# cambridge-mlg/RECOMBINER

Measured on AMD Instinct MI355X. Metric: INRs trained/sec (whole node) + PSNR@bpp vs reference, CIFAR-10, higher is better.
Workload: dtype bf16; 1 GPU; CIFAR-10 32x32, 4096 INRs/GPU, 3x32 SIREN (in 32 = 16 Fourier + 16 upsampled pe), S=1, training_mappings=True, Adam lr 2e-4; inrs_per_gpu=4096, parallelism=datapoint-sharded x1, tuned_library_gemms=True

## Files before the change

include/rcb.h:

```cpp
#ifndef RCB_H_
#define RCB_H_

#include <stdint.h>

#ifdef __cplusplus
extern "C" {
#endif

#define RCB_VERSION 407
#define RCB_OK 0
#define RCB_ERR_ARG (-1)
#define RCB_ERR_SHAPE (-2)
#define RCB_ERR_UNSUPPORTED (-3)
#define RCB_KL_SLOTS 1024
#define RCB_KL_FX_SCALE 16777216.0

typedef void* rcb_stream_t;

int rcb_version(void);
const char* rcb_last_error_string(void);
#define RCB_STRUCT_SIREN_DESC 0
#define RCB_STRUCT_LEVEL 1
#define RCB_STRUCT_LEVEL_BWD 2
#define RCB_STRUCT_ADAM_CFG 3
#define RCB_STRUCT_ADAM_TENSOR 4
#define RCB_STRUCT_REC_DESC 5
int64_t rcb_struct_bytes(int32_t which);

typedef struct {
  int32_t n_rows;
  int32_t samples;
  int32_t n_pix;
// ... 193 lines not shown
} rcb_rec_desc;

int64_t rcb_rec_workspace_bytes(int32_t n_jobs, int32_t max_glen, int32_t n_candidates);
int rcb_rec_score_argmax(const rcb_rec_desc* desc, int32_t mode, void* workspace, int64_t workspace_bytes, int32_t* idx,
                         double* best, uint8_t* uncertified, double* logw_job0, rcb_stream_t stream);
int rcb_rec_commit(const rcb_rec_desc* desc, const int32_t* idx, const int32_t* job_group, int32_t n_groups,
                   double* z_out, float* enc_sample, float* enc_mask, uint8_t* done, float* beta,
                   int32_t* idx_groupwise, rcb_stream_t stream);

int rcb_upconv_fwd(const void* x, int32_t x_is_f32_preact, const float* weff, const float* bias, void* y,
                   int32_t y_is_f32_linear, int32_t batch, int32_t grid, int32_t cout, const void* frag_pack,
                   rcb_stream_t stream);
int32_t rcb_upconv_dgrad_partial_rows(int32_t batch);
int rcb_upconv_dgrad(const void* dy, int32_t dy_is_f32, const float* weff, const void* x, int32_t x_is_f32_preact,
                     void* dx, float* dbias_partial, int32_t batch, int32_t grid, int32_t cout, const void* frag_pack,
                     rcb_stream_t stream);
int64_t rcb_upconv_wgrad_workspace(int32_t batch, int32_t cout);
int rcb_upconv_wgrad(const void* x, int32_t x_is_f32_preact, const void* dy, int32_t dy_is_f32, float* dweff,
                     float* dbias, int32_t batch, int32_t grid, int32_t cout, float* workspace,
                     int64_t workspace_floats, rcb_stream_t stream);
int rcb_upconv_bwd_fused(const void* dy, const float* weff, const void* x, void* dx, float* dweff, float* dbias,
                         int32_t batch, int32_t grid, int32_t cout, float* workspace, int64_t workspace_floats,
                         const void* frag_pack, rcb_stream_t stream);

#define RCB_UPCONV_PACK_UINT4 22528
int rcb_upconv_weff_build(const float* W1, const float* b1, const float* W2, const float* W3, void* weff1, void* b1rep,
                          int32_t bf16_out, float* weff2, float* weff3, void* frag_pack, rcb_stream_t stream);
int rcb_upconv_weff_grad(const void* dweff1, int32_t bf16_in, const float* dweff2, const float* dweff3, float* dW1,
                         float* dW2, float* dW3, const float* db1_partial ,
                         int32_t n_partial, float* db1 ,
                         rcb_stream_t stream);

int rcb_tile_gather(const void* img, void* tiles, int32_t n, int32_t H, int32_t W, int32_t C, int32_t Ty, int32_t Tx,
                    int32_t T, int32_t step, int32_t off, int32_t ring, rcb_stream_t stream);
int rcb_tile_crop(const void* tiles, void* img, int32_t n, int32_t H, int32_t W, int32_t C, int32_t Ty, int32_t Tx,
                  int32_t T, int32_t off, rcb_stream_t stream);
int rcb_tile_fold(const void* tiles, void* img, int32_t n, int32_t H, int32_t W, int32_t C, int32_t Ty, int32_t Tx,
                  int32_t T, int32_t off, rcb_stream_t stream);

int64_t rcb_phaseconv_pack_uint4(int32_t nd, int32_t cout, int32_t which);
int rcb_phaseconv_pack(const float* conv_weight, int32_t nd, int32_t cout, void* fwd_frags, void* dgrad_frags,
                       rcb_stream_t stream);
int rcb_phaseconv_fwd(const void* x, const void* fwd_frags, const float* bias, void* y, int32_t B, int32_t g0, int32_t g1,
                      int32_t g2, int32_t nd, int32_t cout, int32_t leaky_out, rcb_stream_t stream);
int rcb_phaseconv_dgrad(const void* dy, const void* dgrad_frags, const void* x_act, void* dx, int32_t B, int32_t g0,
                        int32_t g1, int32_t g2, int32_t nd, int32_t cout, rcb_stream_t stream);
// ... 27 lines not shown
```

recombiner_amd/_lib.py:

```python
import ctypes as C
import os

import torch

_HERE = os.path.dirname(os.path.abspath(__file__))
LIB_PATH = os.environ.get("RCB_LIB") or os.path.join(_HERE, "lib", "librcb_hip.so")

class RcbError(RuntimeError):
    pass


class SirenDesc(C.Structure):
    _fields_ = [("n_rows", C.c_int32), ("samples", C.c_int32), ("n_pix", C.c_int32), ("fourier_dim", C.c_int32),
                ("pe_dim", C.c_int32), ("n_hidden", C.c_int32), ("hidden", C.c_int32), ("out_dim", C.c_int32),
                ("xf_inr_stride", C.c_int64), ("w_row_stride", C.c_int64), ("w0", C.c_float),
                ("precision", C.c_int32), ("pe_bf16", C.c_int32), ("dw_bf16", C.c_void_p), ("pixel_chunks", C.c_int32),
                ("xf_bf16", C.c_void_p), ("pe_grid_dims", C.c_int32), ("pe_patch_nums", C.c_int32 * 3),
                ("pe_patch_size", C.c_int32 * 3), ("dw_bf16_stride", C.c_int64), ("hidden_dims", C.c_int32 * 4),
                ("dw_lo", C.c_void_p), ("clock_probe", C.c_void_p)]


class Level(C.Structure):
    _fields_ = [("loc", C.c_void_p), ("log_scale", C.c_void_p), ("enc_sample", C.c_void_p),
                ("enc_mask", C.c_void_p), ("row_map", C.c_void_p), ("row_perm", C.c_void_p),
# ... 14 lines not shown


class AdamCfg(C.Structure):
    _fields_ = [("lr", C.c_float), ("beta1", C.c_float), ("beta2", C.c_float), ("eps", C.c_float),
                ("step", C.c_int32), ("dyn_scalars", C.c_void_p)]


class LevelBwd(C.Structure):
    _fields_ = [("loc", C.c_void_p), ("log_scale", C.c_void_p), ("enc_mask", C.c_void_p), ("p_loc", C.c_void_p),
                ("p_scale", C.c_void_p), ("p_scale_is_log", C.c_int32), ("beta", C.c_void_p),
                ("group_idx", C.c_void_p), ("n_groups", C.c_int32), ("kl_scalar", C.c_float),
                ("d_out", C.c_void_p), ("eps", C.c_void_p), ("member_ptr", C.c_void_p),
                ("member_idx", C.c_void_p), ("row_perm_inv", C.c_void_p), ("col_inv", C.c_void_p),
                ("rows", C.c_int32), ("cols", C.c_int32), ("cols_out", C.c_int32), ("samples", C.c_int32),
                ("g_loc", C.c_void_p), ("g_log_scale", C.c_void_p), ("m_loc", C.c_void_p), ("v_loc", C.c_void_p),
                ("m_ls", C.c_void_p), ("v_ls", C.c_void_p), ("kl_accum", C.c_void_p), ("kl_scalar_dev", C.c_void_p),
                ("next_out", C.c_void_p), ("next_eps", C.c_void_p), ("next_out_bf16", C.c_void_p),
                ("next_ld_bf16", C.c_int64), ("rng_seed", C.c_uint64), ("rng_step_dev", C.c_void_p),
                ("rng_step_add", C.c_int64), ("rng_stream", C.c_uint32), ("eps_from_rng", C.c_uint32),
                ("rng_group_offset", C.c_uint64), ("next_out_lo", C.c_void_p), ("sample_sum_ws", C.c_void_p), ("col_map", C.c_void_p)]


_lib = None
ABI_VERSION = 407
_MIRRORS = {0: SirenDesc, 1: Level, 2: LevelBwd, 3: AdamCfg, 4: AdamTensor, 5: RecDesc}

_int, _i32, _i64, _u32, _u64, _f32, _f64, _p = C.c_int, C.c_int32, C.c_int64, C.c_uint32, C.c_uint64, C.c_float, C.c_double, C.c_void_p
_siren, _level, _level_bwd = C.POINTER(SirenDesc), C.POINTER(Level), C.POINTER(LevelBwd)
_adam_cfg, _adam_tensor, _rec = C.POINTER(AdamCfg), C.POINTER(AdamTensor), C.POINTER(RecDesc)
PROTOTYPES = {
    "rcb_version": (_int, []),
    "rcb_last_error_string": (C.c_char_p, []),
    "rcb_struct_bytes": (_i64, [_i32]),
    "rcb_debug_siren_wave_tiles": (_int, [_i32]),
    "rcb_siren_fwd": (_int, [_siren] + [_p] * 5),
    "rcb_siren_bwd": (_int, [_siren] + [_p] * 7),
    "rcb_siren_reduce_chunks": (_int, [_siren] + [_p] * 5),
    "rcb_siren_loss_bwd": (_int, [_siren, _p, _p, _p, _p, _f32, _p, _p, _p, _p]),
    "rcb_reparam_fwd": (_int, [_level, _i32, _i32, _i32, _i32, _p, _p]),
    "rcb_reparam_hier_rng_fwd": (_int, [_level, _i32, _i32, _i32, _p, _p, _u64, _p, _p, _u64, _p]),
    "rcb_philox_normal": (_int, [_p, _i64, _u64, _u32, _p, _i64, _u64, _p]),
    "rcb_reparam_rng_fwd": (_int, [_p, _p, _i64, _u64, _u32, _p, _p, _p, _p, _p, _i32, _i64, _u64, _p]),
    "rcb_gauss_kl": (_int, [_p, _p, _p, _p, _i32, _i32, _i32, _p, _p, _i32, _p, _p, _p, _p, _p]),
    "rcb_gauss_kl_colsum": (_int, [_p, _p, _i32, _p, _p, _i32, _i32, _p, _p]),
    "rcb_beta_update": (_int, [_p, _p, _p, _i32, _i32, _f64, _f64, _f64, _f64, _p]),
    "rcb_posterior_bwd": (_int, [_level_bwd, _adam_cfg, _p]),
    "rcb_adam_flat": (_int, [_p, _p, _p, _p, _i64, _adam_cfg, _p]),
# ... 1 lines not shown
    "rcb_debug_generic_kernels_only": (_int, [_i32]),
    "rcb_atrans_pack_elems": (_i64, [_i32, _p]),
    "rcb_atrans_pack": (_int, [_p, _i32, _p, _p, _i32, _p]),
    "rcb_atrans_plan": (_int, [_i64, _i32, _p, _i32, _p, _i32]),
    "rcb_atrans_apply": (_int, [_p, _i64, _p, _p, _i64, _p, _i64, _i64, _i32, _p, _p, _i32, _i32, _p, _p, _p, _p]),
    "rcb_atrans_workspace_floats": (_i64, [_i64, _i32, _p, _p]),
    "rcb_atrans_wgrad_narrow_workspace": (_i64, [_i32, _i32]),
    "rcb_atrans_wgrad_narrow": (_int, [_p, _p, _p, _i64, _p, _p, _p, _i64, _i64, _i32, _p, _p, _i32, _p]),
    "rcb_step_begin": (_int, [_p, _i64, _p, _p, _p, _p]),
    "rcb_step_end": (_int, [_p, _i32, _f64, _p, _p, _p, _i64, _p, _p, _p]),
    "rcb_step_prepare": (_int, [_p, _i64, _p, _p, _p, _p, _i32, _p, _p, _i32] + [_p] * 6 + [_i32, _p, _p, _p, _p]),
    "rcb_step_tail_eligible": (_int, [_level_bwd]),
    "rcb_step_tail": (_int, [_level_bwd, _adam_cfg, _adam_tensor, _i32, _p, _i32, _f64, _p, _p, _i64, _p, _p, _p, _p]),
    "rcb_col_moments": (_int, [_p, _p, _i32, _i32, _p, _p]),
    "rcb_rec_workspace_bytes": (_i64, [_i32, _i32, _i32]),
    "rcb_rec_score_argmax": (_int, [_rec, _i32, _p, _i64, _p, _p, _p, _p, _p]),
    "rcb_rec_commit": (_int, [_rec, _p, _p, _i32] + [_p] * 7),
    "rcb_upconv_fwd": (_int, [_p, _i32, _p, _p, _p, _i32, _i32, _i32, _i32, _p, _p]),
    "rcb_upconv_dgrad_partial_rows": (_i32, [_i32]),
    "rcb_upconv_dgrad": (_int, [_p, _i32, _p, _p, _i32, _p, _p, _i32, _i32, _i32, _p, _p]),
    "rcb_upconv_wgrad_workspace": (_i64, [_i32, _i32]),
    "rcb_upconv_wgrad": (_int, [_p, _i32, _p, _i32, _p, _p, _i32, _i32, _i32, _p, _i64, _p]),
    "rcb_upconv_bwd_fused": (_int, [_p] * 6 + [_i32, _i32, _i32, _p, _i64, _p, _p]),
    "rcb_upconv_weff_build": (_int, [_p] * 6 + [_i32, _p, _p, _p, _p]),
    "rcb_upconv_weff_grad": (_int, [_p, _i32, _p, _p, _p, _p, _p, _p, _i32, _p, _p]),
    "rcb_tile_gather": (_int, [_p, _p] + [_i32] * 10 + [_p]),
    "rcb_tile_crop": (_int, [_p, _p] + [_i32] * 8 + [_p]),
    "rcb_tile_fold": (_int, [_p, _p] + [_i32] * 8 + [_p]),
    "rcb_phaseconv_pack_uint4": (_i64, [_i32, _i32, _i32]),
    "rcb_phaseconv_pack": (_int, [_p, _i32, _i32, _p, _p, _p]),
    "rcb_phaseconv_fwd": (_int, [_p] * 4 + [_i32] * 7 + [_p]),
    "rcb_phaseconv_dgrad": (_int, [_p] * 4 + [_i32] * 6 + [_p]),
    "rcb_phaseconv_wgrad_workspace": (_i64, [_i32, _i32]),
    "rcb_phaseconv_wgrad": (_int, [_p] * 5 + [_i64] + [_i32] * 6 + [_p]),
    "rcb_stage1_1d_fwd": (_int, [_p, _p, _p, _p, _i32, _i32, _p]),
    "rcb_stage1_1d_dgrad": (_int, [_p, _p, _p, _i32, _i32, _p]),
    "rcb_stage1_1d_wgrad_workspace": (_i64, []),
    "rcb_stage1_1d_wgrad": (_int, [_p] * 5 + [_i64, _i32, _i32, _p]),
    "rcb_window_gather": (_int, [_p, _p] + [_i32] * 6 + [_p]),
    "rcb_window_fold": (_int, [_p, _p] + [_i32] * 6 + [_p]),
    "rcb_phase_bigweight": (_int, [_p, _p, _i32, _i32, _p, _i32, _i32, _i32, _i32, _p]),
    "rcb_phase_bigweight_grad": (_int, [_p, _i32, _p, _i32, _p, _i32, _i32, _i32, _i32, _p]),
    "rcb_softplus_scale": (_int, [_p, _p, _i64, _p]),
}
EXPORTS = list(PROTOTYPES)

# ... 52 lines not shown
```

recombiner_amd/csrc/upconv.hip:

```cpp
#include "rcb_common.h"

using namespace rcb;

typedef float f32x16 __attribute__((ext_vector_type(16)));
typedef __bf16 bf16x8 __attribute__((ext_vector_type(8)));
typedef __bf16 bf16x4 __attribute__((ext_vector_type(4)));
typedef short s16x4 __attribute__((ext_vector_type(4)));

namespace {

constexpr int CIN = 64;
#ifndef RCB_UP_HOT
#define RCB_UP_HOT 0
#endif
#ifndef RCB_UP_NOSTORE
#define RCB_UP_NOSTORE 0
#endif
#ifndef RCB_B3_PF
#define RCB_B3_PF 2
#endif
#ifndef RCB_UP_PF
#define RCB_UP_PF 3
#endif
constexpr int XRS = 72;
// ... 489 lines not shown
#pragma unroll
          for (int k = 0; k < 4; ++k) {
            o0.v[k] = (__bf16)xa[k];     o0.v[4 + k] = (__bf16)ya[k];
            o1.v[k] = (__bf16)xa[4 + k]; o1.v[4 + k] = (__bf16)ya[4 + k];
          }
          uint4* dst = reinterpret_cast<uint4*>(reinterpret_cast<__bf16*>(a.y) + opix * COUT + 32 * mt + 16 * h);
          if (RCB_UP_NOSTORE != 1 || a.batch < 0) {
            dst[0] = o0.u;
            dst[1] = o1.u;
          }
        }
        __builtin_amdgcn_sched_barrier(0);
        F2_T(4);
      }
    }
  }
#if RCB_F2_STAMPS
  ph_[6] = __builtin_amdgcn_s_memrealtime();
  ph_[7] = t_entry_;
  if (blockIdx.x == 0 && lane == 0)
    for (int k = 0; k < 8; ++k) g_f2_stamps[wave * 8 + k] = ph_[k];
#endif
#undef RCB_FETCH2
}

#ifndef RCB_D2_STAMPS
#define RCB_D2_STAMPS 0
#endif
#if RCB_D2_STAMPS
__device__ unsigned long long g_d2_stamps[8 * 8];
#define D2_T(k)                                                     \
  do {                                                              \
    const unsigned long long now_ = __builtin_amdgcn_s_memtime();   \
    ph_[k] += now_ - last_;                                         \
    last_ = now_;                                                   \
  } while (0)
#else
#define D2_T(k) do { } while (0)
#endif
template <int X_F32>
__global__ void __launch_bounds__(512) upconv_dgrad2_reg_kernel(DgradArgs a, float* __restrict__ dbias_partial) {
  constexpr int G = 8, OG = 16, HO = 18, RS = 64, ROWS = HO * RS + 32, COUT = 64, IMG = HO * ROWS;
#if RCB_D2_STAMPS
  const unsigned long long t_entry_ = __builtin_amdgcn_s_memrealtime();
#endif
  extern __shared__ __attribute__((aligned(16))) unsigned char smem_raw[];
// ... 816 lines not shown
}

extern "C" int rcb_upconv_bwd_fused(const void* dy, const float* weff, const void* x, void* dx, float* dweff, float* dbias,
                                    int32_t batch, int32_t grid, int32_t cout, float* workspace, int64_t workspace_floats,
                                    const void* frag_pack, rcb_stream_t stream) {
  RCB_REQUIRE(dy && weff && x && dx && dweff && workspace, RCB_ERR_ARG, "upconv_bwd_fused: null pointer");
  RCB_REQUIRE(batch > 0, RCB_ERR_SHAPE, "upconv_bwd_fused: empty batch");
  RCB_REQUIRE(grid == 16 && cout == 16, RCB_ERR_UNSUPPORTED, "upconv_bwd_fused: grid=%d cout=%d not instantiated", grid, cout);
  RCB_REQUIRE(workspace_floats >= rcb_upconv_wgrad_workspace(batch, cout), RCB_ERR_SHAPE,
              "upconv_bwd_fused: workspace of %lld floats, %lld needed", (long long)workspace_floats,
              (long long)rcb_upconv_wgrad_workspace(batch, cout));
  RCB_REQUIRE((reinterpret_cast<uintptr_t>(frag_pack) & 15) == 0, RCB_ERR_ARG, "upconv_bwd_fused: frag_pack must be 16-byte aligned");
  Bwd3Args a{dy, weff, x, dx, workspace, batch, reinterpret_cast<const uint4*>(frag_pack)};
  hipStream_t st = (hipStream_t)stream;
  const int g = wgrad_blocks(batch);
  static bool done = false;
  int rc = launch(upconv_bwd3_fused_kernel, a, g, 32 * 1024 + (34 * 34 * 24 + 18 * 18 * (RCB_B3_WG16 ? 64 : XRS)) * 2 + 8 * 32 * 40 * 2, st, done);
  if (rc) return rc;
  const int row = 1024 * cout + cout;
  upconv_wgrad_reduce_kernel<<<(row + 63) / 64, 256, 0, st>>>(workspace, g, row, 1024 * cout, dweff, dbias);
  RCB_LAUNCH_CHECK();
  return RCB_OK;
}
```

recombiner_amd/ops.py:

```python
import collections
import ctypes as C
import os as _os
from dataclasses import dataclass
from typing import List, Optional, Sequence

import numpy as np
import torch

from . import _lib
from ._lib import AdamCfg, AdamTensor, Level, LevelBwd, RcbError, SirenDesc, addr, check, ptr, stream_ptr

f32 = torch.float32
f64 = torch.float64
i32 = torch.int32
bf16 = torch.bfloat16


@dataclass(frozen=True)
class SirenMeta:
    samples: int
    n_pix: int
    fourier_dim: int
    pe_dim: int
    n_hidden: int
    hidden: int
    out_dim: int
    w0: float = 30.0
    precision: int = 0
    hidden_dims: Optional[tuple] = None

    @property
    def dims(self):
        hid = list(self.hidden_dims) if self.hidden_dims else [self.hidden] * self.n_hidden
        return [self.fourier_dim + self.pe_dim] + hid + [self.out_dim]

    @property
    def d_net(self):
        dims = self.dims
# ... 829 lines not shown
    jobs, order = RecJobs.from_host(dev, job_row, job_start, job_glen, rows=rows, cols=cols, sort=not want_logw0)
    idx, best, _, logw0 = rec_score(loc, scale, p_loc, p_scale, tables, gumbel, jobs, mode, want_logw0)
    z = rec_commit(p_loc, p_scale, tables, jobs, idx, want_z=True)
    inv = torch.from_numpy(np.argsort(order)).to(dev)
    max_g = int(np.max(job_glen))
    return idx[inv], z[inv][:, :max_g].contiguous(), best[inv], logw0


def _xmode(x, preact):
    if x.dtype == f32:
        return 1
    return 2 if preact else 0


def upconv_fwd(x, weff, bias, grid, cout, out_f32, preact=False, linear_bf16=False, pack=None):
    B = x.shape[0]
    y = torch.empty(B, 2 * grid, 2 * grid, cout, device=x.device, dtype=f32 if out_f32 else bf16)
    omode = 1 if out_f32 else (2 if linear_bf16 else 0)
    _launch("rcb_upconv_fwd", ptr(x), _xmode(x, preact), ptr(weff, f32), ptr(bias, f32), ptr(y), omode, B, grid, cout,
            ptr(pack, None, True))
    return y


def upconv_dgrad(dy, weff, x, grid, cout, preact=False, want_dbias=False, pack=None):
    lib = _lib.load()
    B = x.shape[0]
    dx = torch.empty_like(x)
    part = None
    if want_dbias:
        part = torch.empty(int(lib.rcb_upconv_dgrad_partial_rows(B)), 64, device=x.device, dtype=f32)
    _launch("rcb_upconv_dgrad", ptr(dy), int(dy.dtype == f32), ptr(weff, f32), ptr(x), _xmode(x, preact), ptr(dx),
            ptr(part, f32, True), B, grid, cout, ptr(pack, None, True))
    return (dx, part) if want_dbias else dx


def _wgrad_buffers(lib, B, cout, device):
    buf = torch.empty(2 * 2 * 64 * 2 * 2 * cout + cout, device=device, dtype=f32)
    n_ws = int(lib.rcb_upconv_wgrad_workspace(B, cout))
    return buf[:-cout].view(2, 2, 64, 2, 2, cout), buf[-cout:], torch.empty(n_ws, device=device, dtype=f32), n_ws


def upconv_wgrad(x, dy, grid, cout, preact=False):
    lib = _lib.load()
    B = x.shape[0]
    dw, db, ws, n_ws = _wgrad_buffers(lib, B, cout, x.device)
    _launch("rcb_upconv_wgrad", ptr(x), _xmode(x, preact), ptr(dy), int(dy.dtype == f32), ptr(dw), ptr(db), B, grid, cout,
# ... 378 lines not shown
```

recombiner_amd/prior_model.py:

```python
import os

import numpy as np
import torch
import torch.nn.functional as F
from torch import nn

from . import ops
from . import train_step
from .ops import LevelSpec, SirenMeta
from .upsample_fast import (hip_path_supported, tiled_2d_preferred, phase_form_preferred, phase_module,
                            stitched2d_module, upsample_cifar_hip)
from .utils import count_net_params, hierarchy_row_maps, map_lpe_to_inr_inputs
from .utils import map_hierarchical_model_to_int_weights


class LinearTransform(nn.Module):

    def __init__(self, net_dims):
        super().__init__()
        mats = []
        for i in range(1, len(net_dims)):
            L = net_dims[i] * (net_dims[i - 1] + 1)
            mats.append((torch.rand(L, L) * 2 - 1) / L)
        self.A = nn.ParameterList(mats)
# ... 10 lines not shown
        self.conv2 = conv(64, 64, 3, padding=paddings[1])
        self.conv3 = conv(64, 16, 3, padding=paddings[2])
        self.act1 = nn.LeakyReLU()
        self.up2 = nn.Upsample(scale_factor=layerwise_scale_factors[1])
        self.act2 = nn.LeakyReLU()
        self.up3 = nn.Upsample(scale_factor=layerwise_scale_factors[2])

    def forward(self, x):
        x = self.act1(self.conv1(self.up1(x)))
        x = self.act2(self.conv2(self.up2(x)))
        return self.conv3(self.up3(x))

    def __getstate__(self):
        return {k: v for k, v in self.__dict__.items() if not k.startswith("_rcb_")}


class InrGeometry:

    def _pe_layout(self):
        if self.precision != 0 and self.patch and self.stitched_pe:
            return ops.PeLayout(self.patch_nums[:self.data_dim], self.pixel_sizes[:self.data_dim])
        return None

    def _pe(self, upsample_net, lpe, stitched=False, lpe16=None, weff_cache=None, weight_side_stream=None):
        if self.precision != 0 and hip_path_supported(upsample_net, self.pixel_sizes, self.upsample_factors, self.patch, self.data_dim):
            return upsample_cifar_hip(upsample_net, lpe, self.stage1_bf16, self.pe_bf16, frozen_cache=weff_cache, lpe16=lpe16,
                                      weight_side_stream=weight_side_stream)
        net = upsample_net
        if self.precision != 0 and tiled_2d_preferred(upsample_net, self.patch, self.data_dim):
            net = stitched2d_module(upsample_net)
        elif self.precision != 0 and phase_form_preferred(self.data_dim, self.patch):
            net = phase_module(upsample_net) or upsample_net
        return map_lpe_to_inr_inputs(net, lpe, self.latent_dim, self.pixel_sizes, self.upsample_factors,
                                     self.patch, self.patch_nums, self.data_dim, stitched=stitched)

    def _meta(self, x, pe_dim, samples=1):
        return SirenMeta(samples=samples, n_pix=x.shape[-2], fourier_dim=x.shape[-1], pe_dim=pe_dim,
                         n_hidden=self.n_layers - 1, hidden=max(self.dims[1:-1]), out_dim=self.dims[-1], w0=self.w0,
                         precision=self.precision,
                         hidden_dims=tuple(self.dims[1:-1]) if len(set(self.dims[1:-1])) > 1 else None)

    def _layer_slices(self):
        cum = self.cum_param_sizes
        return [(0 if i == 0 else int(cum[i - 1]), int(cum[i])) for i in range(self.n_layers)]

    def group_to_layer(self, param, layer_idx):
        lo, hi = self._layer_slices()[layer_idx]
        return param[..., lo:hi]


# ... 210 lines not shown
```

recombiner_amd/train_step.py:

```python
import collections
import os
import types

import torch

from . import dist as rdist
from . import ops
from .upsample_fast import hip_path_supported

N_WARM = 3

FORK_A_BACKWARD, FORK_WEIGHT_SIDE, FORK_NET_UPDATE = 2, 4, 8

SWITCHES = ("precision", "patch", "lowp_gemm", "split_gemm", "split_terms", "split_dgrad_terms", "wgrad_bf16", "stage1_bf16",
            "pe_bf16", "fused_noise", "fuse_next_sample", "operand_planes", "redraw_noise", "hier_rng", "rng_row_offset",
            "rng_seed_override", "force_segments", "capture_collectives")
StepPlan = collections.namedtuple("StepPlan", SWITCHES + (
    "n", "n_pix", "n_out", "lr", "training_mappings", "world", "graphable", "fork_mask", "step_fused_env", "posterior_wg_per_cu",
    "lowp", "split", "sharded", "rng_lpe", "use_rng", "rng_hier", "goff_net", "goff_lpe", "want16", "lpe16_want", "fuse_next",
    "fuse_lpe", "planes", "redraw", "redraw_lpe", "pe_stitched", "capture_coll", "one_graph", "update_last", "fork_bwd",
    "fork_wside", "fork_update", "fused_step", "fused_head", "fused_tail"))


def plan_step(model, levels, y, lr, training_mappings, upsample_net, verbose=False):
    m, (net, lpe_lv) = model, levels
    cuda = m.loc.device.type == "cuda"
    D, d_lpe = m._d_net, m._d_lpe
    p = types.SimpleNamespace(**{k: getattr(m, k) for k in SWITCHES})
    N = p.n = y.shape[0]
    p.n_pix, p.n_out = y.shape[1], y.shape[2]
    p.lr, p.training_mappings = float(lr), bool(training_mappings)
    p.world = torch.distributed.get_world_size(m.dp_group) if m.dp_group is not None else 1
    p.graphable = bool(m.use_graph and m.noise_source is None and cuda and not verbose)
    mask = int(os.environ.get("RCB_FORK", str(m.stream_forks)))
    if mask & ~(FORK_A_BACKWARD | FORK_WEIGHT_SIDE | FORK_NET_UPDATE):
        raise ValueError(f"stream_forks / RCB_FORK = {mask}: only combinations of the bits 2 (A-transform backward on a second "
                         "stream), 4 (weight-gradient side of the upsampling net's backward on a third) and 8 (network level's "
                         "posterior update behind the A-transform backward) exist; the orderings behind the bits 1, 16, 32 and "
                         "64 measured no gain or a loss and were removed (DESIGN.md section 4.5 and its round-4 appendix)")
    p.fork_mask = mask if cuda else 0
    p.step_fused_env = os.environ.get("RCB_STEP_FUSED", "1")
    p.posterior_wg_per_cu = os.environ.get("RCB_POSTERIOR_WG_PER_CU", "0")
    p.lowp = bool(m.lowp_gemm and m.precision != 0)
    p.split = bool(m.split_gemm and m.precision != 0 and not m.lowp_gemm)
    p.sharded = bool(p.training_mappings and (p.world > 1 or (m.force_segments and m.dp_group is not None)))
    p.rng_lpe = bool(m.fused_noise and m.noise_source is None and ops.rng_eligible(lpe_lv))
    p.use_rng = bool(p.rng_lpe and len(net) == 1 and ops.rng_eligible(net[0]))
    p.rng_hier = bool(m.hier_rng and p.rng_lpe and not p.use_rng and ops.hier_rng_eligible(net) and (N * D) % 4 == 0
                      and (m.rng_row_offset * D) % 4 == 0)
    p.goff_net = ops.rng_group_offset(m.rng_row_offset, D) if (p.use_rng or p.rng_hier) else 0
    p.goff_lpe = ops.rng_group_offset(m.rng_row_offset, d_lpe) if p.rng_lpe else 0
    p.want16 = bool(p.split and p.training_mappings and m.wgrad_bf16)
    p.lpe16_want = bool(p.use_rng and m.stage1_bf16 and m.precision != 0 and not m.patch)
    p.fuse_next = bool(p.use_rng and m.fuse_next_sample and (N * D) % 4 == 0 and (N * d_lpe) % 4 == 0)
    p.fuse_lpe = bool(p.fuse_next or (p.rng_lpe and m.fuse_next_sample and (N * d_lpe) % 4 == 0))
    p.planes = bool(p.split and p.use_rng and m.operand_planes
                    and all(lo % 8 == 0 for (lo, hi) in m._layer_slices() if (hi - lo) % 8 == 0))
    p.redraw, p.redraw_lpe = bool(p.fuse_next and m.redraw_noise), bool(p.fuse_lpe and m.redraw_noise)
    p.pe_stitched = m._pe_layout() is not None
    p.capture_coll = bool(p.sharded and m.capture_collectives is not False
                          and (m.capture_collectives is True
                               or (torch.distributed.get_backend(m.dp_group) == "nccl" and p.world == 1)))
    p.one_graph = bool(not p.sharded or p.capture_coll)
    p.update_last = bool((p.fuse_next and not p.sharded) or p.capture_coll)
# ... 110 lines not shown
            return {("weff", bool(p.stage1_bf16)): ops.step_prepare(ws["tab"], ws["step_t"], ws["dyn"], ws["kl_slots"], self.split,
                                                                    self.A, c1.weight, c1.bias, c2.weight, c3.weight, p.stage1_bf16)}
        ops.step_begin(ws["tab"], ws["step_t"], ws["dyn"], ws["kl_slots"])
        return None

    def pe_forward(self, weff_cache):
        m, p, N, lpe_lv, rng_ctr = self.model, self.plan, self.plan.n, self.lpe_lv, self.ws["rng_ctr"]
        lpe16 = None
        if p.fuse_lpe:
            smp = self.smp_lpe
            lpe, e_lpe, lpe16 = smp[0], smp[1], (smp[2][:, :lpe_lv.cols] if p.lpe16_want else None)
        elif p.rng_lpe:
            lpe, e_lpe, *o16 = ops.reparam_rng(lpe_lv, self.rng_seed, 1, rng_ctr, want_bf16=p.lpe16_want, group_offset=p.goff_lpe)
            lpe16 = o16[0] if o16 else None
        else:
            e_lpe = m._noise((N, 1, m._d_lpe))
            lpe = ops.reparam_fwd([lpe_lv], [e_lpe], 1)
        lpe_t = lpe.view(1, N, *m._lat, m.latent_dim).requires_grad_(True)
        with torch.enable_grad():
            if self.pe_lay is not None:
                pe_c = m._pe(self.upsample_net, lpe_t, stitched=True)
            else:
                pe = m._pe(self.upsample_net, lpe_t, lpe16=lpe16, weff_cache=weff_cache,
                           weight_side_stream=self.side if p.fork_wside else None)
                pe_c = pe.reshape(N, pe.shape[2], pe.shape[3]).contiguous()
        return lpe_t, e_lpe, pe_c

    def net_forward(self):
        m, p, ws, net, split, A, slices = self.model, self.plan, self.ws, self.net, self.split, self.A, self.slices
        N, D, rng_ctr = p.n, m._d_net, ws["rng_ctr"]
        h16 = A16 = None
        if p.planes:
            if not p.fuse_next:
                ops.reparam_rng(net[0], self.rng_seed, 0, rng_ctr, buffers=self.smp_net, group_offset=p.goff_net)
            h_w, eps = self.smp_net[2], [self.smp_net[1]]
        elif p.fuse_next:
            h_w, e0, h16 = self.smp_net[0], self.smp_net[1], (self.smp_net[2][:, :D] if p.want16 else None)
            eps, h_w = [e0], h_w.view(N, D)
        elif p.use_rng:
            h_w, e0, *o16 = ops.reparam_rng(net[0], self.rng_seed, 0, rng_ctr, want_bf16=p.want16, group_offset=p.goff_net)
            eps, h_w, h16 = [e0], h_w.view(N, D), (o16[0] if o16 else None)
        elif p.rng_hier:
            eps = ws["hier_eps"]
            h_w = ops.reparam_hier_rng(net, eps, self.rng_seed, (0, 2, 3)[:len(net)], rng_ctr, p.goff_net).view(N, D)
        else:
            eps = [m._noise((N, 1, D)) for _ in net]
            h_w = ops.reparam_fwd(net, eps, 1).view(N, D)
# ... 222 lines not shown
```

recombiner_amd/upsample_fast.py:

```python
import itertools
import os
import math

import numpy as np
import torch
import torch.nn.functional as F


def _axis_plan(f: int, k: int, pad: int):
    lo = [min(math.floor((a + kk - pad) / f) for kk in range(k)) for a in range(f)]
    hi = [max(math.floor((a + kk - pad) / f) for kk in range(k)) for a in range(f)]
    w = max(h - l + 1 for l, h in zip(lo, hi))
    pad_l = -min(lo)
    pad_r = max(l + w - 1 for l in lo)
    R = np.zeros([f, w, k], dtype=np.float32)
    for a in range(f):
        for kk in range(k):
            o = math.floor((a + kk - pad) / f)
            R[a, o - lo[a], kk] = 1.0
    shift = [l + pad_l for l in lo]
    return w, pad_l, max(pad_r, 0), shift, R


class PhaseStage:
# ... 330 lines not shown
    return _dev_const("stage1_M", dev, make).to(dtype)


def _phase_R(dev, f, k, pad):
    return _dev_const(("R", f, k, pad), dev, lambda: torch.from_numpy(_axis_plan(f, k, pad)[4]))


def hip_path_supported(net, pixel_sizes, upsample_factors, patch, data_dim):
    try:
        ok = (data_dim == 2 and not patch and list(pixel_sizes) == [32, 32] and list(upsample_factors) == [16, 16]
              and isinstance(net.conv1, torch.nn.Conv2d) and tuple(net.conv1.weight.shape) == (64, 128, 5, 5)
              and tuple(net.conv2.weight.shape) == (64, 64, 3, 3) and tuple(net.conv3.weight.shape) == (16, 64, 3, 3)
              and tuple(net.conv1.padding) == (2, 2) and tuple(net.conv2.padding) == (1, 1)
              and tuple(net.conv3.padding) == (1, 1)
              and [float(net.up1.scale_factor), float(net.up2.scale_factor), float(net.up3.scale_factor)] == [4., 2., 2.])
    except (AttributeError, TypeError):
        ok = False
    return ok


class _UpsampleCifarFn(torch.autograd.Function):

    @staticmethod
    def forward(ctx, lpe, W1, b1, W2, b2, W3, b3, stage1_bf16, pe_bf16, cache=None, lpe16=None, weight_side_stream=None):
        from . import ops
        B = lpe.shape[0]
        ctx.weight_side_stream = weight_side_stream
        key = ("weff", bool(stage1_bf16))
        if cache is not None and key in cache:
            Weff1, b1rep, Weff2, Weff3, pack = cache[key]
        else:
            Weff1, b1rep, Weff2, Weff3, pack = ops.upconv_weff_build(W1, b1, W2, W3, stage1_bf16)
            if cache is not None:
                cache[key] = (Weff1, b1rep, Weff2, Weff3, pack)
        if stage1_bf16:
            lpe = lpe16 if (lpe16 is not None and tuple(lpe16.shape) == tuple(lpe.shape)) else lpe.to(torch.bfloat16)
        z1 = torch.addmm(b1rep, lpe, Weff1).view(B, 8, 8, 64)
        h2 = ops.upconv_fwd(z1, Weff2, b2.contiguous(), 8, 64, out_f32=False, preact=True, pack=pack)
        pe = ops.upconv_fwd(h2, Weff3, b3.contiguous(), 16, 16, out_f32=not pe_bf16, linear_bf16=pe_bf16, pack=pack)
        ctx.save_for_backward(lpe, Weff1, z1, Weff2, h2, Weff3, pack)
        return pe.view(B, 1024, 16)

    @staticmethod
    def backward(ctx, dpe):
        from . import ops
        lpe, Weff1, z1, Weff2, h2, Weff3, pack = ctx.saved_tensors
        B = lpe.shape[0]
        need_w = any(ctx.needs_input_grad[1:7])
        dpe = dpe.contiguous().view(B, 32, 32, 16)
        fused3 = need_w and dpe.dtype == torch.bfloat16
        if fused3:
            dz2, dWeff3, db3 = ops.upconv_bwd_fused(dpe, Weff3, h2, 16, 16, pack=pack)
        else:
            dz2 = ops.upconv_dgrad(dpe, Weff3, h2, 16, 16, pack=pack)
        side = ctx.weight_side_stream if (need_w and fused3) else None
        main = torch.cuda.current_stream() if side is not None else None
        if side is not None:
            side.wait_stream(main)
            with torch.cuda.stream(side):
                dWeff2, db2 = ops.upconv_wgrad(z1, dz2, 8, 64, preact=True)
        dz1, db1_part = ops.upconv_dgrad(dz2, Weff2, z1, 8, 64, preact=True, want_dbias=True, pack=pack)
        dz1f = dz1.view(B, 4096)
        if side is not None:
            side.wait_stream(main)
            with torch.cuda.stream(side):
                dWeff1 = torch.mm(lpe.t(), dz1f, out_dtype=torch.float32) if dz1f.dtype == torch.bfloat16 else lpe.t() @ dz1f
                dW1, dW2, dW3, db1 = ops.upconv_weff_grad(dWeff1, dWeff2, dWeff3, db1_part)
        dlpe = None
        if ctx.needs_input_grad[0]:
            dlpe = torch.mm(dz1f, Weff1.t(), out_dtype=torch.float32) if dz1f.dtype == torch.bfloat16 else dz1f @ Weff1.t()
        if side is not None:
            main.wait_stream(side)
            return dlpe, dW1, db1, dW2, db2, dW3, db3, None, None, None, None, None
        if not need_w:
            return dlpe, None, None, None, None, None, None, None, None, None, None, None
        if not fused3:
            dWeff3, db3 = ops.upconv_wgrad(h2, dpe, 16, 16)
        dWeff2, db2 = ops.upconv_wgrad(z1, dz2, 8, 64, preact=True)
        dWeff1 = (torch.mm(lpe.t(), dz1f, out_dtype=torch.float32) if dz1f.dtype == torch.bfloat16 else lpe.t() @ dz1f)
        dW1, dW2, dW3, db1 = ops.upconv_weff_grad(dWeff1, dWeff2, dWeff3, db1_part)
        return dlpe, dW1, db1, dW2, db2, dW3, db3, None, None, None, None, None


def upsample_cifar_hip(net, lpe, stage1_bf16=True, pe_bf16=True, frozen_cache=None, lpe16=None, weight_side_stream=None):
    S, N = lpe.shape[:2]
    pe = _UpsampleCifarFn.apply(lpe.permute(1, 0, 2, 3, 4).reshape(N * S, 512), net.conv1.weight, net.conv1.bias,
                                net.conv2.weight, net.conv2.bias, net.conv3.weight, net.conv3.bias, bool(stage1_bf16),
                                bool(pe_bf16), frozen_cache, lpe16 if S == 1 else None, weight_side_stream)
    return pe.view(N, S, 1024, 16)


def phase_form_preferred(data_dim, patch):
    return True


def phase_module(net):
    fast = getattr(net, "_rcb_phase_form", None)
    if fast is None:
        try:
            fast = UpsampleFast(net)
            fast.gemm_dtype = torch.bfloat16
        except ValueError:
            fast = False
        object.__setattr__(net, "_rcb_phase_form", fast)
    return fast or None


class _UpsampleStitched23Fn(torch.autograd.Function):

    @staticmethod
    def forward(ctx, z1, W1, b1, W2, b2, W3, b3):
# ... 62 lines not shown
```

Baseline: 74.24 INRs trained/s.

## Fuse upsample conv stages 2 and 3 forward into one producer-consumer kernel

```diff
diff --git a/include/rcb.h b/include/rcb.h
--- a/include/rcb.h
+++ b/include/rcb.h
@@ -7,7 +7,7 @@
 extern "C" {
 #endif
 
-#define RCB_VERSION 407
+#define RCB_VERSION 408
 #define RCB_OK 0
 #define RCB_ERR_ARG (-1)
 #define RCB_ERR_SHAPE (-2)
@@ -247,6 +247,8 @@
 int rcb_upconv_bwd_fused(const void* dy, const float* weff, const void* x, void* dx, float* dweff, float* dbias,
                          int32_t batch, int32_t grid, int32_t cout, float* workspace, int64_t workspace_floats,
                          const void* frag_pack, rcb_stream_t stream);
+int rcb_upconv_fwd23(const void* z1, int32_t z1_is_f32_preact, const float* b2, const float* b3, void* h2, void* pe,
+                     int32_t pe_is_f32_linear, int32_t batch, const void* frag_pack, rcb_stream_t stream);
 
 #define RCB_UPCONV_PACK_UINT4 22528
 int rcb_upconv_weff_build(const float* W1, const float* b1, const float* W2, const float* W3, void* weff1, void* b1rep,
diff --git a/recombiner_amd/_lib.py b/recombiner_amd/_lib.py
--- a/recombiner_amd/_lib.py
+++ b/recombiner_amd/_lib.py
@@ -60,7 +60,7 @@
 
 
 _lib = None
-ABI_VERSION = 407
+ABI_VERSION = 408
 _MIRRORS = {0: SirenDesc, 1: Level, 2: LevelBwd, 3: AdamCfg, 4: AdamTensor, 5: RecDesc}
 
 _int, _i32, _i64, _u32, _u64, _f32, _f64, _p = C.c_int, C.c_int32, C.c_int64, C.c_uint32, C.c_uint64, C.c_float, C.c_double, C.c_void_p
@@ -108,6 +108,7 @@
     "rcb_upconv_wgrad_workspace": (_i64, [_i32, _i32]),
     "rcb_upconv_wgrad": (_int, [_p, _i32, _p, _i32, _p, _p, _i32, _i32, _i32, _p, _i64, _p]),
     "rcb_upconv_bwd_fused": (_int, [_p] * 6 + [_i32, _i32, _i32, _p, _i64, _p, _p]),
+    "rcb_upconv_fwd23": (_int, [_p, _i32, _p, _p, _p, _p, _i32, _i32, _p, _p]),
     "rcb_upconv_weff_build": (_int, [_p] * 6 + [_i32, _p, _p, _p, _p]),
     "rcb_upconv_weff_grad": (_int, [_p, _i32, _p, _p, _p, _p, _p, _p, _i32, _p, _p]),
     "rcb_tile_gather": (_int, [_p, _p] + [_i32] * 10 + [_p]),
diff --git a/recombiner_amd/csrc/upconv.hip b/recombiner_amd/csrc/upconv.hip
--- a/recombiner_amd/csrc/upconv.hip
+++ b/recombiner_amd/csrc/upconv.hip
@@ -535,6 +535,175 @@
     for (int k = 0; k < 8; ++k) g_f2_stamps[wave * 8 + k] = ph_[k];
 #endif
 #undef RCB_FETCH2
+}
+
+struct Fwd23Args {
+  const void* z1;
+  const float* b2;
+  const float* b3;
+  void* h2;
+  void* pe;
+  int batch;
+  const uint4* pack;
+};
+
+__global__ void __launch_bounds__(512) upconv_fwd23_kernel(Fwd23Args a) {
+  constexpr int G = 8, HG = 10, RS = 72, COUT = 64, ZIMG = HG * HG * RS;
+  constexpr int HG3 = 18, RS3 = 64, HIMG = HG3 * HG3 * RS3;
+  extern __shared__ __attribute__((aligned(16))) unsigned char smem_raw[];
+  __bf16* himg = reinterpret_cast<__bf16*>(smem_raw);
+  __bf16* zimg = himg + 2 * HIMG;
+  float* bs = reinterpret_cast<float*>(zimg + 2 * ZIMG);
+  const int tid = threadIdx.x, wave = tid >> 6, lane = tid & 63;
+  const int gs = gridDim.x, b0 = blockIdx.x;
+  const int nloc = b0 < a.batch ? (a.batch - b0 + gs - 1) / gs : 0;
+  for (int e = tid; e < (2 * HIMG + 2 * ZIMG) / 8; e += 512) reinterpret_cast<uint4*>(smem_raw)[e] = make_uint4(0, 0, 0, 0);
+  if (tid < COUT) bs[tid] = a.b2[tid];
+  if (wave < 4) {
+    const int q = lane & 31, h = lane >> 5;
+    const int ph = wave & 3, pa = ph >> 1, pb = ph & 1;
+    uint4 fr[2][2][2][4];
+#pragma unroll
+    for (int mt = 0; mt < 2; ++mt)
+#pragma unroll
+      for (int ty = 0; ty < 2; ++ty)
+#pragma unroll
+        for (int tx = 0; tx < 2; ++tx)
+#pragma unroll
+          for (int kb = 0; kb < 4; ++kb) fr[mt][ty][tx][kb] = a.pack[((((ph * 2 + mt) * 2 + ty) * 2 + tx) * 4 + kb) * 64 + lane];
+#pragma unroll
+    for (int mt = 0; mt < 2; ++mt)
+#pragma unroll
+      for (int ty = 0; ty < 2; ++ty)
+#pragma unroll
+        for (int tx = 0; tx < 2; ++tx)
+#pragma unroll
+          for (int kb = 0; kb < 4; ++kb) pin(fr[mt][ty][tx][kb]);
+    Raw8<3> pre[2];
+#define RCB_FETCH23(bb)                                                                                               \
+  _Pragma("unroll") for (int k_ = 0; k_ < 2; ++k_) pre[k_] = raw_load<3>(a.z1, (long long)(bb) * G * G * CIN + 8 * (tid + 256 * k_));
+#define RCB_COMMIT23(dst)                                                                                             \
+  _Pragma("unroll") for (int k_ = 0; k_ < 2; ++k_) {                                                                  \
+    const int e_ = tid + 256 * k_, pix_ = e_ >> 3, c8_ = e_ & 7;                                                      \
+    Frag f_;                                                                                                          \
+    f_.v = raw_frag<3>(pre[k_], true);                                                                                \
+    *reinterpret_cast<uint4*>((dst) + (((pix_ >> 3) + 1) * HG + ((pix_ & 7) + 1)) * RS + 8 * c8_) = f_.u;             \
+  }
+    if (nloc > 0) RCB_FETCH23(b0)
+    __syncthreads();
+    if (nloc > 0) RCB_COMMIT23(zimg)
+    if (nloc > 1) RCB_FETCH23(b0 + gs)
+    __syncthreads();
+#pragma unroll 1
+    for (int k = 0; k < nloc; ++k) {
+      {
+        const int b = b0 + k * gs;
+        const __bf16* im = zimg + (k & 1) * ZIMG;
+        __bf16* hd = himg + (k & 1) * HIMG;
+#pragma unroll
+        for (int tt = 0; tt < 2; ++tt) {
+          const int pos = tt * 32 + q, i = pos >> 3, j = pos & 7;
+          f32x16 acc[2];
+#pragma unroll
+          for (int mt = 0; mt < 2; ++mt)
+#pragma unroll
+            for (int r = 0; r < 16; ++r) acc[mt][r] = 0.f;
+          const __bf16* base = im + ((i + pa) * HG + (j + pb)) * RS + 8 * h;
+#pragma unroll
+          for (int ty = 0; ty < 2; ++ty)
+#pragma unroll
+            for (int tx = 0; tx < 2; ++tx)
+#pragma unroll
+              for (int kb = 0; kb < 4; ++kb) {
+                Frag bf, fa;
+                bf.u = *reinterpret_cast<const uint4*>(base + (ty * HG + tx) * RS + 16 * kb);
+#pragma unroll
+                for (int mt = 0; mt < 2; ++mt) {
+                  fa.u = fr[mt][ty][tx][kb];
+                  acc[mt] = mfma16(fa.v, bf.v, acc[mt]);
+                }
+              }
+          __builtin_amdgcn_sched_barrier(0);
+          const int oy = 2 * i + pa, ox = 2 * j + pb;
+          const long long opix = ((long long)b * (2 * G) + oy) * (2 * G) + ox;
+          __bf16* hpix = hd + ((oy + 1) * HG3 + (ox + 1)) * RS3;
+          const int sw = ((ox + 1) >> 1) & 7;
+#pragma unroll
+          for (int mt = 0; mt < 2; ++mt) {
+            float v[16];
+#pragma unroll
+            for (int g4 = 0; g4 < 4; ++g4) {
+              const float4 bb = *reinterpret_cast<const float4*>(bs + 32 * mt + 8 * g4 + 4 * h);
+              v[4 * g4 + 0] = lrelu(acc[mt][4 * g4 + 0] + bb.x);
+              v[4 * g4 + 1] = lrelu(acc[mt][4 * g4 + 1] + bb.y);
+              v[4 * g4 + 2] = lrelu(acc[mt][4 * g4 + 2] + bb.z);
+              v[4 * g4 + 3] = lrelu(acc[mt][4 * g4 + 3] + bb.w);
+            }
+            float xa[8], ya[8];
+#pragma unroll
+            for (int m = 0; m < 8; ++m) {
+              auto s2 = __builtin_amdgcn_permlane32_swap(__float_as_uint(v[m]), __float_as_uint(v[8 + m]), false, false);
+              xa[m] = __uint_as_float(s2[0]);
+              ya[m] = __uint_as_float(s2[1]);
+            }
+            Frag o0, o1;
+#pragma unroll
+            for (int kk = 0; kk < 4; ++kk) {
+              o0.v[kk] = (__bf16)xa[kk];     o0.v[4 + kk] = (__bf16)ya[kk];
+              o1.v[kk] = (__bf16)xa[4 + kk]; o1.v[4 + kk] = (__bf16)ya[4 + kk];
+            }
+            uint4* dst = reinterpret_cast<uint4*>(reinterpret_cast<__bf16*>(a.h2) + opix * COUT + 32 * mt + 16 * h);
+            dst[0] = o0.u;
+            dst[1] = o1.u;
+            const int c0 = 4 * mt + 2 * h;
+            *reinterpret_cast<uint4*>(hpix + 8 * (c0 ^ sw)) = o0.u;
+            *reinterpret_cast<uint4*>(hpix + 8 * ((c0 + 1) ^ sw)) = o1.u;
+          }
+          __builtin_amdgcn_sched_barrier(0);
+        }
+      }
+      if (k + 1 < nloc) RCB_COMMIT23(zimg + ((k + 1) & 1) * ZIMG)
+      if (k + 2 < nloc) RCB_FETCH23(b0 + (k + 2) * gs)
+      __syncthreads();
+    }
+    __syncthreads();
+#undef RCB_FETCH23
+#undef RCB_COMMIT23
+  } else {
+    const int w3 = wave - 4, pa = w3 & 1, tp = w3 >> 1;
+    uint4 fr[2][2][2][2];
+#pragma unroll
+    for (int pb = 0; pb < 2; ++pb)
+#pragma unroll
+      for (int ty = 0; ty < 2; ++ty)
+#pragma unroll
+        for (int tx = 0; tx < 2; ++tx)
+#pragma unroll
+          for (int kb2 = 0; kb2 < 2; ++kb2)
+            fr[pb][ty][tx][kb2] = a.pack[16384 + ((((pa * 2 + pb) * 2 + ty) * 2 + tx) * 2 + kb2) * 64 + lane];
+#pragma unroll
+    for (int pb = 0; pb < 2; ++pb)
+#pragma unroll
+      for (int ty = 0; ty < 2; ++ty)
+#pragma unroll
+        for (int tx = 0; tx < 2; ++tx)
+#pragma unroll
+          for (int kb2 = 0; kb2 < 2; ++kb2) pin(fr[pb][ty][tx][kb2]);
+    float bia[4];
+#pragma unroll
+    for (int r = 0; r < 4; ++r) bia[r] = a.b3[4 * (lane >> 4) + r];
+    const FwdArgs a3{nullptr, nullptr, a.b3, a.pe, a.batch, a.pack};
+    __syncthreads();
+    __syncthreads();
+    __syncthreads();
+#pragma unroll 1
+    for (int k = 1; k <= nloc; ++k) {
+      const __bf16* im = himg + ((k - 1) & 1) * HIMG;
+#pragma unroll 1
+      for (int t2 = 0; t2 < 2; ++t2) fwd3_body<16, 1>(im, fr, a3, b0 + (k - 1) * gs, pa, tp + 2 * t2, lane, bia);
+      __syncthreads();
+    }
+  }
 }
 
 #ifndef RCB_D2_STAMPS
@@ -1397,3 +1566,18 @@
   RCB_LAUNCH_CHECK();
   return RCB_OK;
 }
+
+extern "C" int rcb_upconv_fwd23(const void* z1, int32_t z1_is_f32_preact, const float* b2, const float* b3, void* h2, void* pe,
+                                int32_t pe_is_f32_linear, int32_t batch, const void* frag_pack, rcb_stream_t stream) {
+  RCB_REQUIRE(z1 && b2 && b3 && h2 && pe, RCB_ERR_ARG, "upconv_fwd23: null pointer");
+  RCB_REQUIRE(batch > 0, RCB_ERR_SHAPE, "upconv_fwd23: empty batch");
+  RCB_REQUIRE((reinterpret_cast<uintptr_t>(frag_pack) & 15) == 0, RCB_ERR_ARG, "upconv_fwd23: frag_pack must be 16-byte aligned");
+  RCB_REQUIRE(z1_is_f32_preact == 2 && pe_is_f32_linear == 2 && frag_pack, RCB_ERR_UNSUPPORTED,
+              "upconv_fwd23: in_mode=%d out_mode=%d pack=%d: only bf16 pre-activation in, bf16 linear out, with the fragment pack",
+              z1_is_f32_preact, pe_is_f32_linear, frag_pack ? 1 : 0);
+  RCB_REQUIRE(!half_wg(batch), RCB_ERR_UNSUPPORTED, "upconv_fwd23: RCB_UPCONV_HALF_WG=1 keeps the two launches");
+  Fwd23Args a{z1, b2, b3, h2, pe, batch, reinterpret_cast<const uint4*>(frag_pack)};
+  static bool done = false;
+  constexpr int kSmem = 2 * 18 * 18 * 64 * 2 + 2 * 10 * 10 * 72 * 2 + 64 * 4;
+  return launch(upconv_fwd23_kernel, a, batch < 256 ? batch : 256, kSmem, (hipStream_t)stream, done);
+}
diff --git a/recombiner_amd/ops.py b/recombiner_amd/ops.py
--- a/recombiner_amd/ops.py
+++ b/recombiner_amd/ops.py
@@ -14,6 +14,7 @@
 f64 = torch.float64
 i32 = torch.int32
 bf16 = torch.bfloat16
+RCB_ERR_UNSUPPORTED = -3
 
 
 @dataclass(frozen=True)
@@ -889,6 +890,28 @@
     return y
 
 
+def upconv_fwd23_enabled():
+    return _os.environ.get("RCB_UPCONV_FWD_FUSED", "1") != "0"
+
+
+def upconv_fwd23(z1, b2, b3, pack, out=None, pe_f32=False, refuse_ok=False):
+    B = z1.shape[0]
+    if tuple(z1.shape) != (B, 8, 8, 64):
+        raise RcbError(f"upconv_fwd23: z1 must be [B, 8, 8, 64], got {list(z1.shape)}")
+    if out is None:
+        out = (torch.empty(B, 16, 16, 64, device=z1.device, dtype=bf16),
+               torch.empty(B, 32, 32, 16, device=z1.device, dtype=f32 if pe_f32 else bf16))
+    h2, pe = out
+    if tuple(h2.shape) != (B, 16, 16, 64) or h2.dtype != bf16 or tuple(pe.shape) != (B, 32, 32, 16) or pe.dtype not in (f32, bf16):
+        raise RcbError("upconv_fwd23: out must be (bf16 [B, 16, 16, 64], bf16 or fp32 [B, 32, 32, 16])")
+    rc = _lib.load().rcb_upconv_fwd23(ptr(z1), _xmode(z1, True), ptr(b2, f32), ptr(b3, f32), ptr(h2), ptr(pe),
+                                      1 if pe.dtype == f32 else 2, B, ptr(pack, None, True), stream_ptr())
+    if rc == RCB_ERR_UNSUPPORTED and refuse_ok:
+        return None
+    check(rc, "rcb_upconv_fwd23")
+    return h2, pe
+
+
 def upconv_dgrad(dy, weff, x, grid, cout, preact=False, want_dbias=False, pack=None):
     lib = _lib.load()
     B = x.shape[0]
diff --git a/recombiner_amd/prior_model.py b/recombiner_amd/prior_model.py
--- a/recombiner_amd/prior_model.py
+++ b/recombiner_amd/prior_model.py
@@ -56,10 +56,10 @@
             return ops.PeLayout(self.patch_nums[:self.data_dim], self.pixel_sizes[:self.data_dim])
         return None
 
-    def _pe(self, upsample_net, lpe, stitched=False, lpe16=None, weff_cache=None, weight_side_stream=None):
+    def _pe(self, upsample_net, lpe, stitched=False, lpe16=None, weff_cache=None, weight_side_stream=None, fwd_fused=None):
         if self.precision != 0 and hip_path_supported(upsample_net, self.pixel_sizes, self.upsample_factors, self.patch, self.data_dim):
             return upsample_cifar_hip(upsample_net, lpe, self.stage1_bf16, self.pe_bf16, frozen_cache=weff_cache, lpe16=lpe16,
-                                      weight_side_stream=weight_side_stream)
+                                      weight_side_stream=weight_side_stream, fwd_fused=fwd_fused)
         net = upsample_net
         if self.precision != 0 and tiled_2d_preferred(upsample_net, self.patch, self.data_dim):
             net = stitched2d_module(upsample_net)
diff --git a/recombiner_amd/train_step.py b/recombiner_amd/train_step.py
--- a/recombiner_amd/train_step.py
+++ b/recombiner_amd/train_step.py
@@ -16,7 +16,8 @@
             "pe_bf16", "fused_noise", "fuse_next_sample", "operand_planes", "redraw_noise", "hier_rng", "rng_row_offset",
             "rng_seed_override", "force_segments", "capture_collectives")
 StepPlan = collections.namedtuple("StepPlan", SWITCHES + (
-    "n", "n_pix", "n_out", "lr", "training_mappings", "world", "graphable", "fork_mask", "step_fused_env", "posterior_wg_per_cu",
+    "n", "n_pix", "n_out", "lr", "training_mappings", "world", "graphable", "fork_mask", "step_fused_env", "upconv_fwd_fused",
+    "posterior_wg_per_cu",
     "lowp", "split", "sharded", "rng_lpe", "use_rng", "rng_hier", "goff_net", "goff_lpe", "want16", "lpe16_want", "fuse_next",
     "fuse_lpe", "planes", "redraw", "redraw_lpe", "pe_stitched", "capture_coll", "one_graph", "update_last", "fork_bwd",
     "fork_wside", "fork_update", "fused_step", "fused_head", "fused_tail"))
@@ -40,6 +41,7 @@
                          "64 measured no gain or a loss and were removed (DESIGN.md section 4.5 and its round-4 appendix)")
     p.fork_mask = mask if cuda else 0
     p.step_fused_env = os.environ.get("RCB_STEP_FUSED", "1")
+    p.upconv_fwd_fused = bool(ops.upconv_fwd23_enabled())
     p.posterior_wg_per_cu = os.environ.get("RCB_POSTERIOR_WG_PER_CU", "0")
     p.lowp = bool(m.lowp_gemm and m.precision != 0)
     p.split = bool(m.split_gemm and m.precision != 0 and not m.lowp_gemm)
@@ -196,7 +198,7 @@
                 pe_c = m._pe(self.upsample_net, lpe_t, stitched=True)
             else:
                 pe = m._pe(self.upsample_net, lpe_t, lpe16=lpe16, weff_cache=weff_cache,
-                           weight_side_stream=self.side if p.fork_wside else None)
+                           weight_side_stream=self.side if p.fork_wside else None, fwd_fused=p.upconv_fwd_fused)
                 pe_c = pe.reshape(N, pe.shape[2], pe.shape[3]).contiguous()
         return lpe_t, e_lpe, pe_c
 
diff --git a/recombiner_amd/upsample_fast.py b/recombiner_amd/upsample_fast.py
--- a/recombiner_amd/upsample_fast.py
+++ b/recombiner_amd/upsample_fast.py
@@ -376,7 +376,8 @@
 class _UpsampleCifarFn(torch.autograd.Function):
 
     @staticmethod
-    def forward(ctx, lpe, W1, b1, W2, b2, W3, b3, stage1_bf16, pe_bf16, cache=None, lpe16=None, weight_side_stream=None):
+    def forward(ctx, lpe, W1, b1, W2, b2, W3, b3, stage1_bf16, pe_bf16, cache=None, lpe16=None, weight_side_stream=None,
+                fwd_fused=False):
         from . import ops
         B = lpe.shape[0]
         ctx.weight_side_stream = weight_side_stream
@@ -390,8 +391,14 @@
         if stage1_bf16:
             lpe = lpe16 if (lpe16 is not None and tuple(lpe16.shape) == tuple(lpe.shape)) else lpe.to(torch.bfloat16)
         z1 = torch.addmm(b1rep, lpe, Weff1).view(B, 8, 8, 64)
-        h2 = ops.upconv_fwd(z1, Weff2, b2.contiguous(), 8, 64, out_f32=False, preact=True, pack=pack)
-        pe = ops.upconv_fwd(h2, Weff3, b3.contiguous(), 16, 16, out_f32=not pe_bf16, linear_bf16=pe_bf16, pack=pack)
+        out23 = None
+        if fwd_fused and z1.dtype == torch.bfloat16 and pe_bf16 and pack is not None:
+            out23 = ops.upconv_fwd23(z1, b2.contiguous(), b3.contiguous(), pack, refuse_ok=True)
+        if out23 is not None:
+            h2, pe = out23
+        else:
+            h2 = ops.upconv_fwd(z1, Weff2, b2.contiguous(), 8, 64, out_f32=False, preact=True, pack=pack)
+            pe = ops.upconv_fwd(h2, Weff3, b3.contiguous(), 16, 16, out_f32=not pe_bf16, linear_bf16=pe_bf16, pack=pack)
         ctx.save_for_backward(lpe, Weff1, z1, Weff2, h2, Weff3, pack)
         return pe.view(B, 1024, 16)
 
@@ -425,22 +432,28 @@
             dlpe = torch.mm(dz1f, Weff1.t(), out_dtype=torch.float32) if dz1f.dtype == torch.bfloat16 else dz1f @ Weff1.t()
         if side is not None:
             main.wait_stream(side)
-            return dlpe, dW1, db1, dW2, db2, dW3, db3, None, None, None, None, None
+            return dlpe, dW1, db1, dW2, db2, dW3, db3, None, None, None, None, None, None
         if not need_w:
-            return dlpe, None, None, None, None, None, None, None, None, None, None, None
+            return dlpe, None, None, None, None, None, None, None, None, None, None, None, None
         if not fused3:
             dWeff3, db3 = ops.upconv_wgrad(h2, dpe, 16, 16)
         dWeff2, db2 = ops.upconv_wgrad(z1, dz2, 8, 64, preact=True)
         dWeff1 = (torch.mm(lpe.t(), dz1f, out_dtype=torch.float32) if dz1f.dtype == torch.bfloat16 else lpe.t() @ dz1f)
         dW1, dW2, dW3, db1 = ops.upconv_weff_grad(dWeff1, dWeff2, dWeff3, db1_part)
-        return dlpe, dW1, db1, dW2, db2, dW3, db3, None, None, None, None, None
-
-
-def upsample_cifar_hip(net, lpe, stage1_bf16=True, pe_bf16=True, frozen_cache=None, lpe16=None, weight_side_stream=None):
+        return dlpe, dW1, db1, dW2, db2, dW3, db3, None, None, None, None, None, None
+
+
+def upsample_cifar_hip(net, lpe, stage1_bf16=True, pe_bf16=True, frozen_cache=None, lpe16=None, weight_side_stream=None,
+                       fwd_fused=None):
+    from . import ops
+    if fwd_fused is None:
+        fwd_fused = ops.upconv_fwd23_enabled()
+        if frozen_cache is not None:
+            fwd_fused = frozen_cache.setdefault("fwd_fused", fwd_fused)
     S, N = lpe.shape[:2]
     pe = _UpsampleCifarFn.apply(lpe.permute(1, 0, 2, 3, 4).reshape(N * S, 512), net.conv1.weight, net.conv1.bias,
                                 net.conv2.weight, net.conv2.bias, net.conv3.weight, net.conv3.bias, bool(stage1_bf16),
-                                bool(pe_bf16), frozen_cache, lpe16 if S == 1 else None, weight_side_stream)
+                                bool(pe_bf16), frozen_cache, lpe16 if S == 1 else None, weight_side_stream, bool(fwd_fused))
     return pe.view(N, S, 1024, 16)
 
 
```

After: 76.91 INRs trained/s, median of 6. 1.04x the previous value.
